# brianz98/A-Fortran-Electronic-Structure-Program

Measured on AMD Instinct MI355X. Metric: CCSD iter wall-time (s) + (T) wall-time (s); fp64 TFLOP/s vs MFMA peak, higher is better.
Workload: dtype f64; 1 GPU; cfg5: nocc=20 nvirt=200, synthetic hashed ERIs scale 0.005; step = 1 CCSD iteration (replicated) + full (T) over i<=j<=k sharded across ranks; nocc=20, nvirt=200, triples=1540, parallelism=(T) ijk-shard x1, CCSD replicas

## Files before the change

a-fortran-electronic-structure-program_amd/csrc/triples.hip:

```cpp
#include <algorithm>
#include <cmath>
#include <cstdio>
#include <cstdlib>
#include <cstring>
#include <unordered_map>

#include "ccsd.h"
#include "ccsd_so.h"
#include "tgemm.h"
#include "triples_orbit.h"

namespace afesp {

int64_t triples_count(int o) { return (int64_t)o * (o + 1) * (o + 2) / 6; }

__global__ __launch_bounds__(256) void triples_sum_kernel(double* out, const double* partial, int nblk)
{
    __shared__ double sm[4];
    const int q = blockIdx.x;
    const int per = (nblk + (int)gridDim.y - 1) / (int)gridDim.y;
    const int lo = (int)blockIdx.y * per, hi = min(nblk, lo + per);
    double s = 0.0;
    for (int b = lo + threadIdx.x; b < hi; b += blockDim.x) s += partial[(int64_t)q * nblk + b];
#pragma unroll
// ... 80 lines not shown
    for (int off = 32; off > 0; off >>= 1) s += __shfl_down(s, off, 64);
    if ((threadIdx.x & 63) == 0) sm[threadIdx.x >> 6] = s;
    __syncthreads();
    if (threadIdx.x == 0) {
        for (int q = 0; q < 4; ++q) partial[(int64_t)q * nblk_total + blockIdx.x] = 0.0;
        partial[(int64_t)2 * nblk_total + blockIdx.x] = sm[0] + sm[1] + sm[2] + sm[3] + (blockIdx.x == 0 ? 1.0 : 0.0);
    }
}

__global__ __launch_bounds__(256) void triples_build_vt_kernel(double* vt, double* vtT, const double* X, int64_t sb, int64_t sc, int64_t sk,
                                                             int64_t sd, const double* t2, int o, int v, int Kc)
{
    const int64_t n = (int64_t)Kc * v * v * o;
    for (int64_t x = (int64_t)blockIdx.x * blockDim.x + threadIdx.x; x < n; x += (int64_t)gridDim.x * blockDim.x) {
        const int kap = (int)(x % Kc);
        int64_t r = x / Kc;
        const int b = (int)(r % v);
        r /= v;
        const int c = (int)(r % v), k = (int)(r / v);
        double val = 0.0;
        if (kap < v) val = X[sb * b + sc * c + sk * k + sd * kap];
        else if (kap < v + o) val = t2[(kap - v) + (int64_t)o * (k + (int64_t)o * (b + (int64_t)v * c))];
        vt[x] = val;
        vtT[kap + (int64_t)Kc * (c + (int64_t)v * (b + (int64_t)v * k))] = val;
    }
}
__global__ __launch_bounds__(256) void triples_build_vt_tiled_kernel(double* vt, double* vtT, const double* X, int64_t sb, int64_t sk, int64_t sd,
                                                                   const double* t2, int o, int v, int Kc)
{
    __shared__ double tile[32][33];
    const int nkt = (Kc + 31) / 32, nct = (v + 31) / 32;
    int64_t blk = blockIdx.x;
    const int kap0 = (int)(blk % nkt) * 32;
    blk /= nkt;
    const int c0 = (int)(blk % nct) * 32;
    blk /= nct;
    const int b = (int)(blk % v), k = (int)(blk / v);
    const int tx = threadIdx.x & 31, ty = threadIdx.x >> 5;
#pragma unroll
    for (int r = 0; r < 4; ++r) {
        const int kap = kap0 + ty + 8 * r, c = c0 + tx;
        double val = 0.0;
        if (c < v) {
            if (kap < v) val = X[sb * b + c + sk * k + sd * kap];
            else if (kap < v + o) val = t2[(kap - v) + (int64_t)o * (k + (int64_t)o * (b + (int64_t)v * c))];
        }
        tile[ty + 8 * r][tx] = val;
    }
    __syncthreads();
#pragma unroll
    for (int r = 0; r < 4; ++r) {
        const int kap = kap0 + tx, c = c0 + ty + 8 * r;
        if (kap < Kc && c < v) {
            const double val = tile[tx][ty + 8 * r];
            vt[kap + (int64_t)Kc * (b + (int64_t)v * (c + (int64_t)v * k))] = val;
            vtT[kap + (int64_t)Kc * (c + (int64_t)v * (b + (int64_t)v * k))] = val;
        }
    }
}
__global__ __launch_bounds__(256) void triples_build_tt_kernel(double* tt, const double* t2, const double* Y, int64_t si, int64_t sj, int64_t sa,
                                                             int64_t sl, int o, int v, int Kc)
{
    const int64_t n = (int64_t)Kc * v * o * o;
    for (int64_t x = (int64_t)blockIdx.x * blockDim.x + threadIdx.x; x < n; x += (int64_t)gridDim.x * blockDim.x) {
        const int kap = (int)(x % Kc);
        int64_t r = x / Kc;
        const int a = (int)(r % v);
        r /= v;
        const int j = (int)(r % o), i = (int)(r / o);
        double val = 0.0;
        if (kap < v) val = t2[i + (int64_t)o * (j + (int64_t)o * (a + (int64_t)v * kap))];
        else if (kap < v + o) val = -Y[si * i + sj * j + sa * a + sl * (kap - v)];
        tt[x] = val;
    }
}

struct TriplesPlan {
    int o = 0, v = 0;
    int64_t t_begin = -1, t_end = -1, nb = 0;
    int norb = 0;
    bool cr = false;
    int mode = 0;
    int sblock = 0;
    int64_t epoch = -1;
    struct Group { int r; int64_t start, N; int q = 0; int64_t koffA = 0, koffB = 0; };
    struct Chunk { int nt; int64_t meta_off, tab_off, ntab; std::vector<Group> groups;
                   int64_t gdesc_off = 0; int total_tiles = 0, max_ntiles = 0;
                   int64_t gdesc_diag_off = 0; int ngroups_diag = 0, total_tiles_diag = 0, max_ntiles_diag = 0, ngroups_off = 0;
                   int64_t ncol_off = 0, ncol_diag = 0; bool split_diag = false;
                   int64_t tg_off = 0, tab32_off = 0; int tg_ngroups = 0, tg_tiles = 0, tg_max_ntiles = 0; };
    std::vector<Chunk> chunks;
    int64_t* tables = nullptr;
    int64_t off_k = 0, off_Am = 0, off_Cm = 0;
    TripleMeta* meta = nullptr;
    int* orbits = nullptr;
    GettGroup* gdesc = nullptr;
    bool use_tg = false;
    TgGroup* tgdesc = nullptr;
    uint32_t* tables32 = nullptr;
    bool c_pairs = false;
    int k_block = 0;
    int64_t k_pool_gib = -1, k_split_tiles = 0;
    bool k_one_pool = false;
    double* pool0 = nullptr;
};

static std::vector<int64_t> assemble_pool(Context& cx, int64_t nblocks, int64_t vp3, double** pool0)
{
    const size_t bb = (size_t)vp3 * sizeof(double);
    struct Piece { char* base; int64_t n; };
    std::vector<Piece> have;
    int64_t cap = 0;
    for (int i = 0;; ++i) {
        auto it = cx.cache.find("t_xpool" + std::to_string(i));
        if (it == cx.cache.end()) break;
        have.push_back({(char*)it->second.first, (int64_t)(it->second.second / bb)});
        cap += have.back().n;
    }
    if (cap < nblocks) {
        if (!have.empty()) cx.drop_scratch("t_xpool");
        have.clear();
        int64_t need = nblocks;
        for (int i = 0; need > 0; ++i) {
            const std::string name = "t_xpool" + std::to_string(i);
            size_t got = 0;
            void* q = cx.arena.take_largest((size_t)need * bb, (size_t)need * bb + (size_t)need * bb / 4, &got);
            if (!q) q = cx.arena.take_largest((size_t)std::min<int64_t>(need, 8) * bb, (size_t)need * bb, &got);
            int64_t k;
            if (q) {
                k = std::min<int64_t>(need, (int64_t)(got / bb));
                cx.cache[name] = {q, got};
            } else {
                k = need;
                q = cx.scratch(name, k * vp3);
            }
            have.push_back({(char*)q, k});
            need -= k;
        }
    }
    *pool0 = (double*)have[0].base;
    std::vector<int64_t> off;
    off.reserve((size_t)nblocks);
    for (const Piece& pc : have)
        for (int64_t b = 0; b < pc.n && (int64_t)off.size() < nblocks; ++b)
            off.push_back((int64_t)((pc.base - have[0].base) / (ptrdiff_t)sizeof(double)) + b * vp3);
    return off;
}

static bool fused_use_tg(int o, int v);

static TriplesPlan* plan_for(Context& cx, void*& slot, int o, int v, int64_t t_begin, int64_t t_end)
{
    TriplesPlan* p = (TriplesPlan*)slot;
    if (p && p->o == o && p->v == v && p->t_begin == t_begin && p->t_end == t_end && p->mode == 1 && p->epoch == cx.scratch_epoch &&
        p->use_tg == (fused_use_tg(o, v) && (((int64_t)v + o + 15) / 16 * 16) >= 2 * TG_BK))
        return p;
    delete p;
    p = new TriplesPlan();
    slot = p;
    const int64_t O = o, V = v, Kc = (V + O + 15) / 16 * 16;
    p->o = o; p->v = v; p->t_begin = t_begin; p->t_end = t_end; p->cr = false; p->mode = 1;
    p->use_tg = fused_use_tg(o, v) && Kc >= 2 * TG_BK;
    p->c_pairs = (v % 2) == 0;
    std::vector<uint32_t> tab32;
    if (p->use_tg)
        for (int64_t m = 0; m < V * V; ++m) tab32.push_back((uint32_t)(8 * Kc * m));
    const int64_t nt8 = (V + TT - 1) / TT, vp3 = nt8 * nt8 * nt8 * CUBE;
    const int64_t per = 3 * vp3 * (int64_t)sizeof(double);
    size_t mem_free = 0, mem_total = 0;
// ... 122 lines not shown
    cx.sync();
    p->epoch = cx.scratch_epoch;
    return p;
}

static int fused_block_size(int o, int v, bool cr, int64_t budget_bytes)
{
    (void)cr;
    const int64_t nt8 = (v + TT - 1) / TT, vp3 = nt8 * nt8 * nt8 * CUBE;
    const int64_t per_block = vp3 * (int64_t)sizeof(double);
    int smax = 1;
    while (smax < o && (int64_t)3 * (smax + 1) * (smax + 1) * (smax + 1) * per_block <= budget_bytes) ++smax;
    if (knobs().t_block > 0) return std::max(1, std::min(smax, knobs().t_block));
    const int smin = std::min(smax, std::max(1, (900 + v - 1) / v));
    auto fill = [&](int sz) { return (double)((int64_t)v * sz) / (double)((((int64_t)v * sz + 127) / 128) * 128); };
    int best = smin;
    for (int sz = smin + 1; sz <= std::min(smax, smin + 2); ++sz)
        if (fill(sz) > fill(best) + 0.02) best = sz;
    return best;
}

static int64_t device_pool_budget()
{
    size_t mem_free = 0, mem_total = 0;
    AFESP_HIP(hipMemGetInfo(&mem_free, &mem_total));
    if (knobs().t_pool_gib >= 0) return knobs().t_pool_gib << 30;
    return std::min<int64_t>((int64_t)64 << 30, (int64_t)(mem_total / 4));
}

static bool fused_use_tg(int o, int v)
{
    if (knobs().t_gemm_gett) return false;
    const int64_t O = o, V = v, Kc = (V + O + 15) / 16 * 16;
    return 8 * Kc * V * V < ((int64_t)1 << 32) && 8 * Kc * V * O * O < ((int64_t)1 << 32);
}

static TriplesPlan* plan_fused(Context& cx, void*& slot, int o, int v, int64_t t_begin, int64_t t_end, bool cr)
{
    TriplesPlan* p = (TriplesPlan*)slot;
    const bool use_tg = fused_use_tg(o, v);
    if (p && p->o == o && p->v == v && p->t_begin == t_begin && p->t_end == t_end && p->cr == cr && p->mode == 0 &&
        p->epoch == cx.scratch_epoch && p->use_tg == use_tg && p->k_block == knobs().t_block && p->k_pool_gib == knobs().t_pool_gib &&
        p->k_split_tiles == knobs().t_split_tiles && p->k_one_pool == knobs().t_one_pool)
        return p;
    delete p;
    p = new TriplesPlan();
    slot = p;
    const int64_t O = o, V = v, v2 = V * V, Kc = (V + O + 15) / 16 * 16;
    const int64_t nt8 = (V + TT - 1) / TT, vp3 = nt8 * nt8 * nt8 * CUBE;
    p->o = o; p->v = v; p->t_begin = t_begin; p->t_end = t_end; p->cr = cr; p->mode = 0; p->use_tg = use_tg;
    p->k_block = knobs().t_block; p->k_pool_gib = knobs().t_pool_gib; p->k_split_tiles = knobs().t_split_tiles; p->k_one_pool = knobs().t_one_pool;
    p->c_pairs = (v % 2) == 0;
    const int nk1 = (int)(Kc / TG_BK);
    std::vector<uint32_t> tab32;
    if (use_tg)
        for (int64_t m = 0; m < v2; ++m) tab32.push_back((uint32_t)(8 * Kc * m));
    const int sb = fused_block_size(o, v, cr, device_pool_budget());
    p->sblock = sb;
    const int nbk = (o + sb - 1) / sb;
    std::vector<int64_t> tab;
    p->off_k = 0;
    p->off_Am = (int64_t)tab.size();
    for (int64_t c = 0; c < V; ++c)
        for (int64_t b = 0; b < V; ++b) tab.push_back(Kc * (b + V * c));
    p->off_Cm = (int64_t)tab.size();
    for (int64_t c = 0; c < V; ++c)
        for (int64_t b = 0; b < V; ++b)
            tab.push_back(CUBE * nt8 * (b / TT) + TT * (b % TT) + CUBE * nt8 * nt8 * (c / TT) + TT * TT * (c % TT));
    std::vector<TripleMeta> metas;
    int64_t flat = 0, max_blocks = 1;
    int tm, tn, BM, BN;
    gett_grouped_tile((int)v2, true, &tm, &tn, &BM, &BN);
    const int mtiles = (int)((v2 + BM - 1) / BM);
    const int64_t split_min_tiles = knobs().t_split_tiles;
    {
        int64_t fl = 0;
        for (int I = 0; I < nbk; ++I)
            for (int J = I; J < nbk; ++J)
                for (int K = J; K < nbk; ++K) {
                    std::unordered_map<int64_t, int> seen;
                    for (int i = I * sb; i < std::min(o, (I + 1) * sb); ++i)
                        for (int j = std::max(i, J * sb); j < std::min(o, (J + 1) * sb); ++j)
                            for (int k = std::max(j, K * sb); k < std::min(o, (K + 1) * sb); ++k, ++fl) {
                                if (fl < t_begin || fl >= t_end) continue;
                                const int pq[3][3] = {{i, j, k}, {j, i, k}, {k, i, j}};
                                for (auto& b : pq) seen.emplace(((int64_t)b[0] * o + std::min(b[1], b[2])) * o + std::max(b[1], b[2]), 0);
                            }
                    max_blocks = std::max<int64_t>(max_blocks, (int64_t)seen.size());
                }
    }
    if (cr) {
        if (cx.cache.count("t_xpool0")) cx.drop_scratch("t_xpool");
    } else {
        cx.drop_scratch("t_mpool");
        if (cx.cache.count("t_xpool")) {
            cx.quiesce();
            cx.arena.put(cx.cache["t_xpool"].first);
            cx.cache.erase("t_xpool");
            ++cx.scratch_epoch;
        }
    }
    std::vector<int64_t> blk_off;
    if (cr || knobs().t_one_pool) {
        for (int64_t b = 0; b < max_blocks; ++b) blk_off.push_back(b * vp3);
        p->pool0 = nullptr;
    } else {
        blk_off = assemble_pool(cx, max_blocks, vp3, &p->pool0);
    }
    for (int I = 0; I < nbk; ++I)
        for (int J = I; J < nbk; ++J)
            for (int K = J; K < nbk; ++K) {
                std::vector<TripleMeta> cur;
                struct Blk { int p, q, r; int64_t buf; };
                std::vector<Blk> blks;
                std::unordered_map<int64_t, int64_t> seen;
                auto block_of = [&](int pp, int qq, int rr) {
                    if (qq > rr) std::swap(qq, rr);
                    const int64_t key = ((int64_t)pp * o + qq) * o + rr;
                    auto it = seen.find(key);
                    if (it != seen.end()) return it->second;
                    blks.push_back({pp, qq, rr, (int64_t)blks.size()});
                    seen.emplace(key, blks.back().buf);
                    return blks.back().buf;
                };
                for (int i = I * sb; i < std::min(o, (I + 1) * sb); ++i)
                    for (int j = std::max(i, J * sb); j < std::min(o, (J + 1) * sb); ++j)
                        for (int k = std::max(j, K * sb); k < std::min(o, (K + 1) * sb); ++k, ++flat) {
                            if (flat < t_begin || flat >= t_end) continue;
                            TripleMeta m;
                            m.i = i; m.j = j; m.k = k;
                            m.pad = (j == k ? 1 : 0) | (i == k ? 2 : 0) | (i == j ? 4 : 0);
                            m.mult = (i == j && j == k) ? 1.0 : (i == j || j == k) ? 3.0 : 6.0;
                            m.woff = 0;
                            for (int q = 0; q < 6; ++q) m.xoff[q] = 0;
                            m.xoff[0] = blk_off[(size_t)block_of(i, j, k)];
                            m.xoff[1] = blk_off[(size_t)block_of(j, i, k)];
                            m.xoff[5] = blk_off[(size_t)block_of(k, i, j)];
                            cur.push_back(m);
                        }
                if (cur.empty()) continue;
                TriplesPlan::Chunk ch;
                ch.nt = (int)cur.size();
                ch.meta_off = (int64_t)metas.size();
                metas.insert(metas.end(), cur.begin(), cur.end());
                if ((int64_t)blks.size() > max_blocks) throw Error(2, "triples plan: block count of a chunk exceeds the pool");
                std::vector<int64_t> hBn, hCn, hK;
                std::stable_sort(blks.begin(), blks.end(), [](const Blk& x, const Blk& y) { return x.q != y.q ? x.q < y.q : x.r < y.r; });
                for (size_t b0 = 0; b0 < blks.size();) {
                    const int q = blks[b0].q, r = blks[b0].r;
                    size_t b1 = b0;
                    while (b1 < blks.size() && blks[b1].q == q && blks[b1].r == r) ++b1;
                    const int64_t start = (int64_t)hBn.size();
                    for (size_t bi = b0; bi < b1; ++bi)
                        for (int64_t x = 0; x < V; ++x) {
                            hBn.push_back(Kc * (x + V * (q + O * blks[bi].p)));
                            hCn.push_back(CUBE * (x / TT) + x % TT + blk_off[(size_t)blks[bi].buf]);
                        }
                    b0 = b1;
                    TriplesPlan::Group g;
                    g.r = r; g.q = q; g.start = start; g.N = (int64_t)hBn.size() - start;
                    g.koffA = (int64_t)hK.size();
                    for (int64_t x = 0; x < Kc; ++x) hK.push_back(x);
                    for (int64_t x = 0; x < Kc; ++x) hK.push_back(Kc * v2 * O + Kc * v2 * ((int64_t)q - r) + x);
                    g.koffB = (int64_t)hK.size();
                    for (int64_t x = 0; x < Kc; ++x) hK.push_back(x);
                    for (int64_t x = 0; x < Kc; ++x) hK.push_back(Kc * V * ((int64_t)r - q) + x);
                    ch.groups.push_back(g);
                }
                int64_t diag_tiles = 0;
                for (const TriplesPlan::Group& g : ch.groups)
                    if (g.q == g.r) diag_tiles += mtiles * ((g.N + BN - 1) / BN);
                ch.split_diag = diag_tiles >= split_min_tiles;
                if (use_tg) ch.split_diag = nk1 >= 2;
                if (!ch.split_diag)
                    for (int t = 0; t < ch.nt; ++t) metas[ch.meta_off + t].pad = 0;
                ch.ntab = (int64_t)hBn.size();
                if (use_tg) {
                    ch.tab32_off = (int64_t)tab32.size();
                    for (int64_t x : hBn) tab32.push_back((uint32_t)(8 * x));
                }
                ch.tab_off = (int64_t)tab.size();
                tab.insert(tab.end(), hBn.begin(), hBn.end());
                tab.insert(tab.end(), hCn.begin(), hCn.end());
                const int64_t kbase = (int64_t)tab.size() - ch.tab_off;
                tab.insert(tab.end(), hK.begin(), hK.end());
                for (TriplesPlan::Group& g : ch.groups) { g.koffA += kbase; g.koffB += kbase; }
                p->chunks.push_back(std::move(ch));
            }
    p->nb = max_blocks;
    std::vector<int> orb;
    for (int A = 0; A < nt8; ++A)
        for (int B = A; B < nt8; ++B)
            for (int C = B; C < nt8; ++C) orb.push_back(A | (B << 10) | (C << 20));
    p->norb = (int)orb.size();
    if (metas.empty()) metas.push_back(TripleMeta());
    tab.resize(tab.size() + 128, 0);
    p->tables = (int64_t*)cx.scratch("t_tables", (int64_t)tab.size());
    p->meta = (TripleMeta*)cx.scratch("t_meta", (int64_t)(metas.size() * sizeof(TripleMeta) / sizeof(double) + 1));
    p->orbits = (int*)cx.scratch("t_orbits", (int64_t)orb.size() / 2 + 1);
    AFESP_HIP(hipMemcpyAsync(p->tables, tab.data(), tab.size() * sizeof(int64_t), hipMemcpyHostToDevice, cx.stream));
    AFESP_HIP(hipMemcpyAsync(p->meta, metas.data(), metas.size() * sizeof(TripleMeta), hipMemcpyHostToDevice, cx.stream));
    AFESP_HIP(hipMemcpyAsync(p->orbits, orb.data(), orb.size() * sizeof(int), hipMemcpyHostToDevice, cx.stream));
    std::vector<GettGroup> gd;
    for (TriplesPlan::Chunk& ch : p->chunks) {
        const int64_t* tabs = p->tables + ch.tab_off;
      for (int diag = 0; diag < 2; ++diag) {
        (diag ? ch.gdesc_diag_off : ch.gdesc_off) = (int64_t)gd.size();
        int tile = 0, ng = 0, mx = 0;
        int64_t ncol = 0;
        for (const TriplesPlan::Group& g : ch.groups) {
            if ((ch.split_diag && g.q == g.r) != (diag == 1)) continue;
            GettGroup d;
            d.a_off = Kc * v2 * g.r;
            d.offAk = tabs + g.koffA;
            d.offBk = tabs + g.koffB;
            d.offBn = tabs + g.start;
            d.offCn = tabs + ch.ntab + g.start;
            d.N = (int)g.N;
            d.ntiles = (int)((g.N + BN - 1) / BN);
            d.tile_start = tile;
            d.pad = 0;
            tile += mtiles * d.ntiles;
            mx = std::max(mx, d.ntiles);
            ncol += g.N;
            ++ng;
            gd.push_back(d);
        }
        GettGroup end{};
        end.tile_start = tile;
        gd.push_back(end);
        if (diag) { ch.total_tiles_diag = tile; ch.ngroups_diag = ng; ch.max_ntiles_diag = mx; ch.ncol_diag = ncol; }
        else { ch.total_tiles = tile; ch.ngroups_off = ng; ch.max_ntiles = mx; ch.ncol_off = ncol; }
      }
    }
    p->gdesc = (GettGroup*)cx.scratch("t_gdesc", (int64_t)(gd.size() * sizeof(GettGroup) / sizeof(double) + 1));
    AFESP_HIP(hipMemcpyAsync(p->gdesc, gd.data(), gd.size() * sizeof(GettGroup), hipMemcpyHostToDevice, cx.stream));
    std::vector<TgGroup> tg;
    if (use_tg) {
        tab32.resize(tab32.size() + 256, 0u);
        p->tables32 = (uint32_t*)cx.scratch("t_tables32", (int64_t)(tab32.size() / 2 + 1));
        AFESP_HIP(hipMemcpyAsync(p->tables32, tab32.data(), tab32.size() * sizeof(uint32_t), hipMemcpyHostToDevice, cx.stream));
        const int mt = (int)((v2 + TG_BM - 1) / TG_BM);
        for (TriplesPlan::Chunk& ch : p->chunks) {
            const int64_t* tabs = p->tables + ch.tab_off;
            ch.tg_off = (int64_t)tg.size();
            int mx = 0;
            for (const TriplesPlan::Group& g : ch.groups) mx = std::max(mx, (int)((g.N + TG_BN - 1) / TG_BN));
            const int gm = tgemm_group_m((int)v2, mx);
            int tile = 0;
            for (int pass = 0; pass < 2; ++pass)
            for (const TriplesPlan::Group& g : ch.groups) {
                const bool half = ch.split_diag && g.q == g.r;
                if (half != (pass == 1)) continue;
                TgGroup d;
                d.a1 = Kc * v2 * g.r;
                d.a2 = Kc * v2 * O + Kc * v2 * g.q;
                d.b1 = 0;
                d.b2 = Kc * V * ((int64_t)g.r - g.q);
                d.c0 = 0;
                d.colB = p->tables32 + ch.tab32_off + g.start;
                d.offCn = tabs + ch.ntab + g.start;
                d.N = (int)g.N;
                d.ntiles = (int)((g.N + TG_BN - 1) / TG_BN);
                d.tile_start = tile;
                d.nk1 = nk1;
                d.nk = half ? nk1 : 2 * nk1;
                d.inv_width = tgemm_inverse(gm * d.ntiles);
                if ((int64_t)mt * d.ntiles * gm * d.ntiles >= ((int64_t)1 << 32)) throw Error(2, "triples plan: tile walk out of range");
                tile += mt * d.ntiles;
                tg.push_back(d);
            }
            TgGroup end{};
            end.tile_start = tile;
            tg.push_back(end);
            ch.tg_ngroups = (int)ch.groups.size();
            ch.tg_tiles = tile;
            ch.tg_max_ntiles = mx;
        }
        p->tgdesc = (TgGroup*)cx.scratch("t_tgdesc", (int64_t)(tg.size() * sizeof(TgGroup) / sizeof(double) + 1));
        AFESP_HIP(hipMemcpyAsync(p->tgdesc, tg.data(), tg.size() * sizeof(TgGroup), hipMemcpyHostToDevice, cx.stream));
    }
    cx.sync();
    p->epoch = cx.scratch_epoch;
    return p;
}

static double fused_range_cost(int o, int v, int sb, int64_t b, int64_t e, int BM, int BN, int64_t split_min_tiles)
{
    const int64_t V = v, O = o, v2 = V * V, Kc = (V + O + 15) / 16 * 16;
    const int64_t nt8 = (V + TT - 1) / TT, vp3 = nt8 * nt8 * nt8 * CUBE;
    const int64_t mtiles = (v2 + BM - 1) / BM;
    const int nbk = (o + sb - 1) / sb;
    const double half_tile_s = 2.0 * BM * BN * (double)Kc / 58e12;
    const double triple_s = 3.0 * (double)vp3 * 8.0 / 3.9e12;
    double cost = 0.0;
    int64_t flat = 0;
    std::unordered_map<int64_t, int> npair;
    std::unordered_map<int64_t, char> seen;
    for (int I = 0; I < nbk && flat < e; ++I)
        for (int J = I; J < nbk && flat < e; ++J)
            for (int K = J; K < nbk && flat < e; ++K) {
                npair.clear();
                seen.clear();
                int64_t nt = 0;
                auto need = [&](int pp, int qq, int rr) {
                    if (qq > rr) std::swap(qq, rr);
                    if (seen.emplace(((int64_t)pp * o + qq) * o + rr, 1).second) ++npair[(int64_t)qq * o + rr];
                };
                for (int i = I * sb; i < std::min(o, (I + 1) * sb); ++i)
                    for (int j = std::max(i, J * sb); j < std::min(o, (J + 1) * sb); ++j)
                        for (int k = std::max(j, K * sb); k < std::min(o, (K + 1) * sb); ++k, ++flat) {
                            if (flat < b || flat >= e) continue;
                            ++nt;
                            need(i, j, k);
                            need(j, i, k);
                            need(k, i, j);
                        }
                if (nt == 0) continue;
                int64_t off = 0, diag = 0;
                for (const auto& g : npair) {
                    const int64_t tiles = mtiles * ((V * g.second + BN - 1) / BN);
                    (g.first / o == g.first % o ? diag : off) += tiles;
                }
                const double halves = 2.0 * (double)off + (diag >= split_min_tiles ? 1.0 : 2.0) * (double)diag;
                cost += std::max(halves, 512.0) * half_tile_s + (double)nt * triple_s + 40e-6;
            }
    return cost;
}

void triples_shard_bounds(int o, int v, bool cr, int world, int64_t* bounds)
{
    const int64_t V = v, nt = triples_count(o);
    int tm, tn, BM, BN;
    gett_grouped_tile((int)(V * V), true, &tm, &tn, &BM, &BN);
    const int sb = fused_block_size(o, v, cr, device_pool_budget());
    const int64_t split_min_tiles = knobs().t_split_tiles;
    auto cost = [&](int64_t b, int64_t e) { return fused_range_cost(o, v, sb, b, e, BM, BN, split_min_tiles); };
    bounds[0] = 0;
    if (cost(0, nt) < (double)world * cost(0, 1)) {
        for (int r = 1; r <= world; ++r) bounds[r] = nt * r / world;
        return;
    }
    for (int r = 0; r < world; ++r) {
        const int64_t b = bounds[r];
        if (r == world - 1 || b >= nt) { bounds[r + 1] = nt; continue; }
        const double target = cost(b, nt) / (double)(world - r);
        int64_t lo = b, hi = nt;
        while (lo < hi) {
            const int64_t mid = (lo + hi) / 2;
            if (cost(b, mid) >= target) hi = mid; else lo = mid + 1;
        }
        if (lo > b + 1 && target - cost(b, lo - 1) < cost(b, lo) - target) --lo;
        bounds[r + 1] = lo;
    }
}

int triples_block_size(int o, int v, bool cr) { return fused_block_size(o, v, cr, device_pool_budget()); }

void triples_plan_free(CCState& s)
{
    delete (TriplesPlan*)s.tplan;
    s.tplan = nullptr;
}

void ccsd_triples(Context& cx, CCState& s, int64_t t_begin, int64_t t_end, double* out_host, bool cr, bool want_d)
{
    if (cr) want_d = true;
    if (cr && !s.have_cr) throw Error(1, "ccsd_triples: completely renormalised mode needs ccsd_cr_intermediates first");
    if (!s.ready) throw Error(1, "ccsd_triples: no converged CCSD state in this context");
    const int o = s.o, v = s.v;
    const int64_t O = o, V = v, v2 = V * V, v3 = V * V * V;
    const int64_t nt8 = (V + TT - 1) / TT, vp3 = nt8 * nt8 * nt8 * CUBE;
    const int64_t Kc = (V + O + 15) / 16 * 16;
    t_begin = std::max<int64_t>(0, t_begin);
    t_end = std::min<int64_t>(triples_count(o), t_end);
    TriplesPlan* p = plan_fused(cx, s.tplan, s.o, s.v, t_begin, t_end, cr);
    if (knobs().t_debug)
        fprintf(stderr, "afesp (T): o %d v %d block %d chunks %zu kernel %s\n", o, v, p->sblock, p->chunks.size(), p->use_tg ? "tgemm" : "gett");
    Tensor vt = view(cx.scratch("t_vt", 2 * Kc * v2 * O), {Kc, V, V, O}), tt = view(cx.scratch("t_tt", Kc * V * O * O), {Kc, V, O, O});
    Tensor vtT = vt;
    vtT.d = vt.d + Kc * v2 * O;
    auto blocks = [](int64_t n) { return dim3((unsigned)std::min<int64_t>((n + 255) / 256, 65536)); };
    const bool ops_valid = cx.t_ops_owner == (const void*)&s && cx.t_ops_amp == s.amp_epoch && cx.t_ops_scratch == cx.scratch_epoch;
    if (!ops_valid) { cx.t_ops_ts = false; cx.t_ops_cr = -1; }
    if (!ops_valid) {
        const int64_t nblk = ((Kc + 31) / 32) * ((V + 31) / 32) * V * O;
        if (nblk < ((int64_t)1 << 31))
            AFESP_KLAUNCH(triples_build_vt_tiled_kernel, dim3((unsigned)nblk), dim3(256), 0, cx.stream, vt.d, vtT.d, s.v_vvov.d, V, v2,
                               v2 * O, s.t2.d, o, v, (int)Kc);
        else
            AFESP_KLAUNCH(triples_build_vt_kernel, blocks(Kc * v2 * O), dim3(256), 0, cx.stream, vt.d, vtT.d, s.v_vvov.d, V,
                               (int64_t)1, v2, v2 * O, s.t2.d, o, v, (int)Kc);
        AFESP_HIP(hipGetLastError());
        AFESP_KLAUNCH(triples_build_tt_kernel, blocks(Kc * V * O * O), dim3(256), 0, cx.stream, tt.d, s.t2.d, s.v_oovo.d, (int64_t)1, O,
                           O * O, O * O * V, o, v, (int)Kc);
        AFESP_HIP(hipGetLastError());
    }
    Tensor vs = view(cx.scratch("t_vs", v2 * O * O), {V, V, O, O});
    Tensor ts = view(cx.scratch("t_ts", v2 * O * O), {V, V, O, O});
    if (!ops_valid) permute_add(cx, 1.0, s.v_oovv, "pqxy", 0.0, vs, "xypq");
    if (want_d && !cx.t_ops_ts) {
        permute_add(cx, 1.0, s.t2, "pqxy", 0.0, ts, "xypq");
        cx.t_ops_ts = true;
    }
    Tensor vt2, tt2;
    double* Mpool = nullptr;
    if (cr) {
        vt2 = view(cx.scratch("t_vt2", 2 * Kc * v2 * O), {Kc, V, V, O});
        tt2 = view(cx.scratch("t_tt2", Kc * V * O * O), {Kc, V, O, O});
        Tensor vt2T = vt2;
        vt2T.d = vt2.d + Kc * v2 * O;
        if (cx.t_ops_cr != s.cr_epoch) {
            AFESP_KLAUNCH(triples_build_vt_kernel, blocks(Kc * v2 * O), dim3(256), 0, cx.stream, vt2.d, vt2T.d, s.I_vovv_pp.d, V * O,
                               v2 * O, V, (int64_t)1, s.t2.d, o, v, (int)Kc);
            AFESP_HIP(hipGetLastError());
            AFESP_KLAUNCH(triples_build_tt_kernel, blocks(Kc * V * O * O), dim3(256), 0, cx.stream, tt2.d, s.t2.d, s.I_ooov_pp.d, O,
                               (int64_t)1, O * O * O, O * O, o, v, (int)Kc);
            AFESP_HIP(hipGetLastError());
            cx.t_ops_cr = s.cr_epoch;
        }
        Mpool = cx.scratch("t_mpool", p->nb * vp3);
    }
    cx.t_ops_owner = (const void*)&s;
    cx.t_ops_amp = s.amp_epoch;
    cx.t_ops_scratch = cx.scratch_epoch;
    const int nq = cr ? 6 : want_d ? 4 : 2;
    const bool dbase = t_begin == 0 && want_d;
    double pub_seq = 0.0;
    double* pub = (p->chunks.size() == 1 && !dbase && (int64_t)p->norb * p->chunks[0].nt <= 8192) ? host_scalars_slot(cx, &pub_seq) : nullptr;
    if (!pub) k_fill(cx, cx.scal, 6, 0.0);
    TriplesIn in{s.e, s.t1.d, vs.d, ts.d, s.t2.d, o, v};
    double* Xpool = p->pool0 ? p->pool0 : cx.scratch("t_xpool", p->nb * vp3);
    int64_t max_nt = 1;
    for (const TriplesPlan::Chunk& ch : p->chunks) max_nt = std::max<int64_t>(max_nt, ch.nt);
    double* partial = cx.scratch("t_partial", 6 * std::max<int64_t>((int64_t)p->norb * max_nt, 512));
    double* sum_tmp = cx.scratch("t_sum_tmp", 6 * 128);
    std::vector<hipEvent_t> evs;
    auto stamp = [&]() {
        if (!cx.prof) return;
        hipEvent_t e;
        AFESP_HIP(hipEventCreate(&e));
        AFESP_HIP(hipEventRecord(e, cx.stream));
        evs.push_back(e);
    };
    for (const TriplesPlan::Chunk& ch : p->chunks) {
        stamp();
        {
            GettProblem gp;
            gp.A = vt.d;
            gp.B = tt.d;
            gp.C = Xpool;
            gp.offAm = p->tables + p->off_Am;
            gp.offAk = gp.offBk = gp.offBn = gp.offCn = nullptr;
            gp.offCm = p->tables + p->off_Cm;
            gp.M = (int)v2; gp.N = 0; gp.K = (int)(2 * Kc);
            gp.alpha = 1.0; gp.beta = 0.0;
            gp.nbatch = 1; gp.batchA = gp.batchB = gp.batchC = nullptr;
            gp.a_kcontig = gp.b_kcontig = true;
            gp.wide = true;
            GettProblem gm = gp;
            gm.A = vt2.d;
            gm.B = tt2.d;
            gm.C = Mpool;
            if (p->use_tg) {
                TgProblem tp{vt.d, tt.d, Xpool, p->tables32, p->tables + p->off_Cm, (int)v2, p->c_pairs, (int)((V + O - (Kc - TG_BK) + 3) / 4)};
                AFESP_HIP(tgemm_launch(tp, p->tgdesc + ch.tg_off, ch.tg_ngroups, ch.tg_tiles, ch.tg_max_ntiles, cx.stream, cx.tg));
                if (cr) {
                    TgProblem tm{vt2.d, tt2.d, Mpool, p->tables32, p->tables + p->off_Cm, (int)v2, p->c_pairs, (int)((V + O - (Kc - TG_BK) + 3) / 4)};
                    AFESP_HIP(tgemm_launch(tm, p->tgdesc + ch.tg_off, ch.tg_ngroups, ch.tg_tiles, ch.tg_max_ntiles, cx.stream, cx.tg));
                }
            } else {
            if (ch.ngroups_off > 0) {
                const GettGroup* gd = p->gdesc + ch.gdesc_off;
                AFESP_HIP(gett_launch_grouped(gp, gd, ch.ngroups_off, ch.total_tiles, ch.max_ntiles, cx.stream));
                if (cr) AFESP_HIP(gett_launch_grouped(gm, gd, ch.ngroups_off, ch.total_tiles, ch.max_ntiles, cx.stream));
            }
            if (ch.ngroups_diag > 0) {
                const GettGroup* gd = p->gdesc + ch.gdesc_diag_off;
                gp.K = gm.K = (int)Kc;
                AFESP_HIP(gett_launch_grouped(gp, gd, ch.ngroups_diag, ch.total_tiles_diag, ch.max_ntiles_diag, cx.stream));
                if (cr) AFESP_HIP(gett_launch_grouped(gm, gd, ch.ngroups_diag, ch.total_tiles_diag, ch.max_ntiles_diag, cx.stream));
            }
            }
            if (cx.prof) {
                cx.prof_gemm_kind = p->use_tg ? 1 : 0;
                for (const TriplesPlan::Group& g : ch.groups) {
                    const bool half = ch.split_diag && g.q == g.r;
                    if (p->use_tg) {
                        const double kexec = (double)(Kc - TG_BK) + ((V + O - (Kc - TG_BK) + 3) / 4 < 4 ? 12.0 : 16.0);
                        cx.prof_gemm_flop_padded += 2.0 * (double)((v2 + TG_BM - 1) / TG_BM * TG_BM) * (double)((g.N + TG_BN - 1) / TG_BN * TG_BN) *
                                                    kexec * (half ? 1.0 : 2.0);
                    } else {
                        int tm_, tn_, BM_, BN_;
                        gett_grouped_tile((int)v2, true, &tm_, &tn_, &BM_, &BN_);
                        cx.prof_gemm_flop_padded += 2.0 * (double)((v2 + BM_ - 1) / BM_ * BM_) * (double)((g.N + BN_ - 1) / BN_ * BN_) *
                                                    (double)Kc * (half ? 1.0 : 2.0);
                    }
                }
                cx.prof_gemm_launches += p->use_tg ? 1 : (ch.ngroups_off > 0) + (ch.ngroups_diag > 0);
                cx.prof_gemm_flop += 2.0 * (double)gp.M * (double)(2 * ch.ncol_off + ch.ncol_diag) * (double)(V + O);
            }
        }
        stamp();
        if (cr)
            AFESP_KLAUNCH((triples_orbit_kernel<true, true>), dim3(p->norb, ch.nt), dim3(256), 0, cx.stream, partial, Xpool, Mpool,
                               p->meta + ch.meta_off, p->orbits, in, p->norb * ch.nt);
        else if (!want_d)
            AFESP_KLAUNCH((triples_orbit_kernel<false, true, false>), dim3(p->norb, ch.nt), dim3(256), 0, cx.stream, partial, Xpool,
                               Mpool, p->meta + ch.meta_off, p->orbits, in, p->norb * ch.nt);
        else
            AFESP_KLAUNCH((triples_orbit_kernel<false, true>), dim3(p->norb, ch.nt), dim3(256), 0, cx.stream, partial, Xpool, Mpool,
                               p->meta + ch.meta_off, p->orbits, in, p->norb * ch.nt);
        AFESP_HIP(hipGetLastError());
        stamp();
        if (cx.prof) {
            cx.prof_orbit_launches += 1;
            cx.prof_orbit_bytes += 8.0 * 3.0 * (double)v3 * ch.nt;
        }
        if (pub) {
            AFESP_KLAUNCH(triples_sum_publish_kernel, dim3(1), dim3(256), 0, cx.stream, cx.scal, pub, pub_seq, partial, nq, p->norb * ch.nt);
            AFESP_HIP(hipGetLastError());
        } else {
            sum_partials(cx, cx.scal, partial, nq, p->norb * ch.nt, sum_tmp);
        }
    }
    if (dbase) {
        AFESP_KLAUNCH(triples_dbase_kernel, dim3(256), dim3(256), 0, cx.stream, partial, in, 256);
        AFESP_HIP(hipGetLastError());
        AFESP_KLAUNCH(triples_sum_kernel, dim3(4), dim3(256), 0, cx.stream, cx.scal, partial, 256);
        AFESP_HIP(hipGetLastError());
    }
    double* h = pub ? host_scalars_wait(cx, 6, pub_seq) : host_scalars(cx, 6);
    if (!evs.empty()) AFESP_HIP(hipEventSynchronize(evs.back()));
    for (size_t q = 0; q + 2 < evs.size(); q += 3) {
        float a = 0.f, b = 0.f;
        AFESP_HIP(hipEventElapsedTime(&a, evs[q], evs[q + 1]));
        AFESP_HIP(hipEventElapsedTime(&b, evs[q + 1], evs[q + 2]));
        cx.prof_gemm_ms += a;
        cx.prof_orbit_ms += b;
    }
    for (hipEvent_t e : evs) (void)hipEventDestroy(e);
    out_host[0] = h[0];
    out_host[1] = h[0] + h[1];
    if (!want_d) return;
    out_host[2] = h[2];
    out_host[3] = h[2] + h[3];
    if (cr) {
        out_host[4] = h[4];
        out_host[5] = h[4] + h[5];
    }
}

int64_t so_triples_count(int o) { return (int64_t)o * (o - 1) * (o - 2) / 6; }

void so_triples_plan_free(SOState& s)
{
    delete (TriplesPlan*)s.tplan;
    s.tplan = nullptr;
}

__global__ void so_levels_kernel(double* e_so, const double* e, int n2)
{
    const int x = blockIdx.x * blockDim.x + threadIdx.x;
    if (x < n2) e_so[x] = e[x / 2];
}

double so_triples(Context& cx, SOState& s, int64_t t_begin, int64_t t_end)
{
    if (!s.ready) throw Error(1, "ccsd_so_triples: no converged spin-orbital CCSD state in this context");
    if (s.fock && s.f_offdiag > 1e-8)
        throw Error(1, "ccsd_so_triples: the occupied-occupied / virtual-virtual Fock blocks of this state are not diagonal (largest off-diagonal "
                       "element " + std::to_string(s.f_offdiag) + "): (T) needs semicanonical orbitals");
    const int o = s.o, v = s.v;
    const int64_t O = o, V = v, v2 = V * V;
    const int64_t nt8 = (V + TT - 1) / TT, vp3 = nt8 * nt8 * nt8 * CUBE;
    const int64_t Kc = (V + O + 15) / 16 * 16;
    t_begin = std::max<int64_t>(0, t_begin);
    t_end = std::min<int64_t>(so_triples_count(o), t_end);
    k_fill(cx, cx.scal, 1, 0.0);
    if (t_end <= t_begin) return 0.0;
    TriplesPlan* p = plan_for(cx, s.tplan, o, v, t_begin, t_end);
    Tensor vt = view(cx.scratch("t_vt", Kc * v2 * O), {Kc, V, V, O}), tt = view(cx.scratch("t_tt", Kc * V * O * O), {Kc, V, O, O});
    Tensor vs = view(cx.scratch("t_vs", v2 * O * O), {V, V, O, O});
    double* e_so = cx.scratch("t_eso", O + V);
    const bool ops_valid = cx.t_ops_owner == (const void*)&s && cx.t_ops_amp == s.amp_epoch && cx.t_ops_scratch == cx.scratch_epoch;
    if (!ops_valid) {
    auto sub = [&](const Tensor& full, int64_t row0, int64_t nrows) {
        Tensor t = full;
        t.d = full.d + row0;
        t.dim[0] = nrows;
        return t;
    };
    if (Kc != V + O) {
        AFESP_HIP(hipMemsetAsync(vt.d, 0, sizeof(double) * Kc * v2 * O, cx.stream));
        AFESP_HIP(hipMemsetAsync(tt.d, 0, sizeof(double) * Kc * V * O * O, cx.stream));
    }
    permute_add(cx, 1.0, s.vovv, "fpbc", 0.0, sub(vt, 0, V), "fbcp");
    permute_add(cx, 1.0, s.t2, "mpcb", 0.0, sub(vt, V, O), "mbcp");
    permute_add(cx, 1.0, s.t2, "qraf", 0.0, sub(tt, 0, V), "farq");
    permute_add(cx, -1.0, s.ovoo, "maqr", 0.0, sub(tt, V, O), "marq");
// ... 65 lines not shown
```

a-fortran-electronic-structure-program_amd/csrc/triples_orbit.h:

```cpp
#pragma once
#include <hip/hip_runtime.h>
#include <stdint.h>

namespace afesp {

struct TripleMeta {
    int i, j, k, pad;
    double mult;
    int64_t xoff[6];
    int64_t woff;
};

struct TriplesIn {
    const double* e;
    const double* t1;
    const double* voovv_s;
    const double* t2_s;
    const double* t2;
    int o, v;
};

#ifdef AFESP_ORBIT_STAMPS
constexpr int ORB_SLOTS = 4096;
__device__ unsigned long long g_orbit_stamp[ORB_SLOTS * 16];
#define ORB_STAMP(k)                                                                                                          \
    {                                                                                                                         \
        const unsigned long long now_ = __builtin_amdgcn_s_memtime();                                                         \
        if (threadIdx.x == 0) g_orbit_stamp[((blockIdx.y * gridDim.x + blockIdx.x) % ORB_SLOTS) * 16 + (k)] = now_ - orb_last_; \
        orb_last_ = now_;                                                                                                     \
    }
#else
#define ORB_STAMP(k) {}
#endif

#ifndef AFESP_ORBIT_DEPTH
#define AFESP_ORBIT_DEPTH 0
#endif
constexpr int TT = 8;
constexpr int CUBE = TT * TT * TT;
constexpr int PATCH = TT * TT;

__host__ __device__ constexpr int sig(int s, int d)
{
    return s == 0 ? d : s == 1 ? (d == 0 ? 1 : d == 1 ? 0 : 2) : s == 2 ? 2 - d : s == 3 ? (d == 0 ? 0 : d == 1 ? 2 : 1)
                      : s == 4 ? (d + 1) % 3 : (d + 2) % 3;
}
__device__ __forceinline__ double rcp_nr(double x)
{
    double r = __builtin_amdgcn_rcp(x);
    r = __builtin_fma(__builtin_fma(-x, r, 1.0), r, r);
    r = __builtin_fma(__builtin_fma(-x, r, 1.0), r, r);
    return r;
}
__device__ __forceinline__ int cidx(int p0, int p1, int p2) { return ((p0 ^ p1 ^ p2) & 7) | (p1 << 3) | (p2 << 6); }

__host__ __device__ constexpr int orbit_term(bool fused, int idx) { return fused ? (idx == 0 ? 0 : idx == 1 ? 1 : 5) : idx; }

__host__ __device__ constexpr int compose(int q, int s)
{
    for (int r = 0; r < 6; ++r)
        if (sig(r, 0) == sig(q, sig(s, 0)) && sig(r, 1) == sig(q, sig(s, 1)) && sig(r, 2) == sig(q, sig(s, 2))) return r;
    return 0;
}

template <bool CR, bool FUSED, bool WANT_D = true>
__global__ __launch_bounds__(256, CR ? 2 : WANT_D ? 3 : 4) void triples_orbit_kernel(double* __restrict__ partial, const double* __restrict__ Xpool,
                                                            const double* __restrict__ Mpool,
                                                            const TripleMeta* __restrict__ meta,
                                                            const int* __restrict__ orbits, TriplesIn in, int nblk_total)
{
    __shared__ __attribute__((aligned(16))) double stage[6 * CUBE];
    __shared__ double vp[27 * PATCH];
    __shared__ double tp[WANT_D ? 27 * PATCH : 1];
    __shared__ double t1r[96];
    __shared__ int srcq[6][6];
    __shared__ double red[24];
#ifdef AFESP_ORBIT_STAMPS
    unsigned long long orb_last_ = __builtin_amdgcn_s_memtime();
#endif
    const TripleMeta m = meta[blockIdx.y];
    const int o = in.o, v = in.v, t = threadIdx.x;
    const int packed = orbits[blockIdx.x];
    const int tile[3] = {packed & 1023, (packed >> 10) & 1023, (packed >> 20) & 1023};
    if (t < 36) {
        const int s = t / 6, q = t % 6;
        int want[3];
        for (int d = 0; d < 3; ++d) want[d] = tile[sig(q, sig(s, d))];
        int found = 0;
        for (int r = 5; r >= 0; --r)
            if (tile[sig(r, 0)] == want[0] && tile[sig(r, 1)] == want[1] && tile[sig(r, 2)] == want[2]) found = r;
        srcq[s][q] = found;
    }
    const int64_t vv = (int64_t)v * v;
    const int l0 = t & 7, l1 = (t >> 3) & 7, l2h[2] = {t >> 6, (t >> 6) + 4};
    const int nt8 = (v + TT - 1) / TT;
    const int p0 = (2 * t) & 7, p1 = (t >> 2) & 7, p2 = t >> 5;
    const int sbase = (((p0 ^ p1 ^ p2) & 7) & ~1) | (p1 << 3) | (p2 << 6);
    const bool flip = ((p1 ^ p2) & 1) != 0;
    typedef double v2d_t __attribute__((ext_vector_type(2)));
    auto load_term = [&](const double* X, v2d_t (&xin)[6]) {
#pragma unroll
        for (int q = 0; q < 6; ++q) {
            const int T0 = tile[sig(q, 0)], T1 = tile[sig(q, 1)], T2 = tile[sig(q, 2)];
            const v2d_t x = *reinterpret_cast<const v2d_t*>(X + (int64_t)CUBE * (T0 + (int64_t)nt8 * (T1 + (int64_t)nt8 * T2)) + 2 * t);
            const int g0 = T0 * TT + p0;
            const bool rows = (T1 * TT + p1 < v) && (T2 * TT + p2 < v);
            xin[q][0] = (rows && g0 < v) ? x[0] : 0.0;
            xin[q][1] = (rows && g0 + 1 < v) ? x[1] : 0.0;
        }
    };
    auto park_term = [&](const v2d_t (&xin)[6]) {
#pragma unroll
        for (int q = 0; q < 6; ++q)
            *reinterpret_cast<v2d_t*>(&stage[q * CUBE + sbase]) = flip ? (v2d_t){xin[q][1], xin[q][0]} : xin[q];
    };
    constexpr int NT1 = FUSED ? 3 : 6;
    constexpr int NTERM = CR ? 2 * NT1 : NT1;
    constexpr int DEPTH = AFESP_ORBIT_DEPTH > 0 ? (AFESP_ORBIT_DEPTH < NT1 ? AFESP_ORBIT_DEPTH : NT1) : CR ? 3 : 2;
    v2d_t xin[DEPTH][6];
#pragma unroll
    for (int s2 = 0; s2 < DEPTH; ++s2) load_term(Xpool + m.xoff[orbit_term(FUSED, s2)], xin[s2]);
    const int occ[3] = {m.i, m.j, m.k};
    const int pairp[3] = {m.j, m.i, m.i}, pairq[3] = {m.k, m.k, m.j};
    {
        const int g = __builtin_amdgcn_readfirstlane(t >> 6), loc = t & 63;
#pragma unroll
        for (int i = 0; i < 5; ++i) {
            const int P = g + 4 * i;
            if (P < 18) {
                const int pr = P / 6, pi = P % 6;
                const int sx = pi < 2 ? 0 : pi < 4 ? 1 : 2, sy = pi == 0 ? 1 : pi == 1 ? 2 : pi == 2 ? 0 : pi == 3 ? 2 : pi == 4 ? 0 : 1;
                const int gx = tile[sx] * TT + (loc & 7), gy = tile[sy] * TT + (loc >> 3);
                const bool ok = gx < v && gy < v;
                const int64_t off = (ok ? gx + (int64_t)v * gy : 0) + vv * (pairp[pr] + (int64_t)o * pairq[pr]);
                const int dst = (pr * 9 + sx * 3 + sy) * PATCH + loc;
                const double a = in.voovv_s[off];
                vp[dst] = ok ? a : 0.0;
                if (WANT_D) {
                    const double b = in.t2_s[off];
                    tp[dst] = ok ? b : 0.0;
                }
            }
        }
    }
    if (t < 72) {
        const int oc = t / 24, sl = (t / 8) % 3, l = t & 7, g = tile[sl] * TT + l;
        t1r[t] = g < v ? in.t1[occ[oc] + o * g] : 0.0;
    } else if (t < 96) {
        const int sl = (t - 72) / 8, l = t & 7, g = tile[sl] * TT + l;
        t1r[t] = in.e[(g < v ? g : 0) + o];
    }
    const double* evl = t1r + 72;
    double wreg[12];
    double mreg[CR ? 12 : 1];
#pragma unroll
    for (int r = 0; r < 12; ++r) wreg[r] = 0.0;
#pragma unroll
    for (int r = 0; r < (CR ? 12 : 1); ++r) mreg[r] = 0.0;
#pragma unroll
    for (int s2 = 0; s2 < NTERM; ++s2) {
        const int s = orbit_term(FUSED, s2 % NT1);
        const int sT = s == 0 ? 3 : s == 1 ? 4 : 2;
        const bool sym = FUSED && ((m.pad >> (s2 % NT1)) & 1);
        if (s2 == 0) ORB_STAMP(0)
        __syncthreads();
        park_term(xin[s2 % DEPTH]);
        if (s2 + DEPTH < NTERM)
            load_term((s2 + DEPTH < NT1 ? Xpool : Mpool) + m.xoff[orbit_term(FUSED, (s2 + DEPTH) % NT1)], xin[s2 % DEPTH]);
        __syncthreads();
        if (s2 < 3) ORB_STAMP(1 + 2 * s2)
#define ORB_READ(sg) stage[srcq[sg][q] * CUBE + cidx(l[sig(q, sig(sg, 0))], l[sig(q, sig(sg, 1))], l[sig(q, sig(sg, 2))])]
        double xr[12];
        if (FUSED && sym) {
#pragma unroll
            for (int r = 0; r < 12; ++r) {
                const int q = r >> 1;
                const int l[3] = {l0, l1, l2h[r & 1]};
                xr[r] = ORB_READ(s) + ORB_READ(sT);
            }
        } else {
#pragma unroll
            for (int r = 0; r < 12; ++r) {
                const int q = r >> 1;
                const int l[3] = {l0, l1, l2h[r & 1]};
                xr[r] = ORB_READ(s);
            }
        }
#undef ORB_READ
#pragma unroll
        for (int r = 0; r < 12; ++r) {
            if (s2 < NT1) wreg[r] += xr[r];
            else mreg[CR ? r : 0] += xr[r];
        }
        if (s2 < 3) ORB_STAMP(2 + 2 * s2)
    }
    const double eo = in.e[m.i] + in.e[m.j] + in.e[m.k];
    constexpr int NQ = CR ? 6 : WANT_D ? 4 : 2;
    double acc[NQ];
#pragma unroll
    for (int q = 0; q < NQ; ++q) acc[q] = 0.0;
#pragma unroll
    for (int h = 0; h < 2; ++h) {
        int l2v = l2h[h];
        if (h == 1) asm volatile("" : "+v"(l2v) : "v"(acc[0]), "v"(acc[NQ - 1]));
        const int l[3] = {l0, l1, l2v};
        const bool live = tile[0] * TT + l[0] < v && tile[1] * TT + l[1] < v && tile[2] * TT + l[2] < v;
        const double D = eo - evl[l[0]] - evl[TT + l[1]] - evl[2 * TT + l[2]];
        const double rD = rcp_nr(3.0 * D);
        const double r3D = live ? rD : 0.0;
        double t1v[3][3], Z[6], Y[WANT_D ? 6 : 1];
#pragma unroll
        for (int oc = 0; oc < 3; ++oc)
#pragma unroll
            for (int c = 0; c < 3; ++c) t1v[oc][c] = t1r[oc * 24 + c * TT + l[c]];
        {
            double V[3][3][3];
#pragma unroll
            for (int pr = 0; pr < 3; ++pr)
#pragma unroll
                for (int cx = 0; cx < 3; ++cx)
#pragma unroll
                    for (int cy = 0; cy < 3; ++cy)
                        if (cx != cy) V[pr][cx][cy] = vp[(pr * 9 + cx * 3 + cy) * PATCH + l[cx] + TT * l[cy]];
#pragma unroll
            for (int q = 0; q < 6; ++q) {
                const int s0 = sig(q, 0), s1 = sig(q, 1), s2 = sig(q, 2);
                Z[q] = t1v[0][s0] * V[0][s1][s2] + t1v[1][s1] * V[1][s0][s2] + t1v[2][s2] * V[2][s0][s1];
            }
        }
        if (WANT_D) {
            int lt[3] = {l[0], l[1], l[2]};
            asm volatile("" : "+v"(lt[0]), "+v"(lt[1]), "+v"(lt[2]) : "v"(Z[0]), "v"(Z[1]), "v"(Z[2]), "v"(Z[3]), "v"(Z[4]), "v"(Z[5]));
            double T2[3][3][3];
#pragma unroll
            for (int pr = 0; pr < 3; ++pr)
#pragma unroll
                for (int cx = 0; cx < 3; ++cx)
#pragma unroll
                    for (int cy = 0; cy < 3; ++cy)
                        if (cx != cy) T2[pr][cx][cy] = tp[(pr * 9 + cx * 3 + cy) * PATCH + lt[cx] + TT * lt[cy]];
#pragma unroll
            for (int q = 0; q < 6; ++q) {
                const int s0 = sig(q, 0), s1 = sig(q, 1), s2 = sig(q, 2);
                Y[q] = t1v[0][s0] * t1v[1][s1] * t1v[2][s2] + t1v[0][s0] * T2[0][s1][s2] + t1v[1][s1] * T2[1][s0][s2] +
                       t1v[2][s2] * T2[2][s0][s1];
            }
        }
#pragma unroll
        for (int q = 0; q < 6; ++q) {
            const double w = wreg[2 * q + h];
#define BAR3(A) (4.0 * A(q) + A(compose(q, 4)) + A(compose(q, 5)) - 2.0 * (A(compose(q, 3)) + A(compose(q, 1)) + A(compose(q, 2))))
#define W_AT(r) wreg[2 * (r) + h]
// ... 181 lines not shown
```

Measured before the change: 59.74 TFLOP/s.

## Skip i=j=k triples and reuse staged orbit terms for duplicate occupied indices

Drops fully diagonal (i=j=k) triples from the plan, partitioning and pool sizing, since their contribution is treated as zero. In the fused orbit kernel, triples with i==j or j==k now skip loading and staging the duplicate term: the already-parked shared-memory stage is reused and the register prefetch pipeline is shifted. This removes redundant global loads and barrier pairs for degenerate triples, at the cost of more complex per-block control flow and pointer selection. It also guards against empty host-to-device copies and adjusts partition cost and debug output.

```diff
diff --git a/a-fortran-electronic-structure-program_amd/csrc/triples.hip b/a-fortran-electronic-structure-program_amd/csrc/triples.hip
--- a/a-fortran-electronic-structure-program_amd/csrc/triples.hip
+++ b/a-fortran-electronic-structure-program_amd/csrc/triples.hip
@@ -186,9 +186,11 @@
     bool cr = false;
     int mode = 0;
     int sblock = 0;
+    int nblock_triples = 0;
     int64_t epoch = -1;
     struct Group { int r; int64_t start, N; int q = 0; int64_t koffA = 0, koffB = 0; };
-    struct Chunk { int nt; int64_t meta_off, tab_off, ntab; std::vector<Group> groups;
+    struct Chunk { int nt; int ndup = 0;
+                   int64_t meta_off, tab_off, ntab; std::vector<Group> groups;
                    int64_t gdesc_off = 0; int total_tiles = 0, max_ntiles = 0;
                    int64_t gdesc_diag_off = 0; int ngroups_diag = 0, total_tiles_diag = 0, max_ntiles_diag = 0, ngroups_off = 0;
                    int64_t ncol_off = 0, ncol_diag = 0; bool split_diag = false;
@@ -477,7 +479,7 @@
                     for (int i = I * sb; i < std::min(o, (I + 1) * sb); ++i)
                         for (int j = std::max(i, J * sb); j < std::min(o, (J + 1) * sb); ++j)
                             for (int k = std::max(j, K * sb); k < std::min(o, (K + 1) * sb); ++k, ++fl) {
-                                if (fl < t_begin || fl >= t_end) continue;
+                                if (fl < t_begin || fl >= t_end || (i == j && j == k)) continue;
                                 const int pq[3][3] = {{i, j, k}, {j, i, k}, {k, i, j}};
                                 for (auto& b : pq) seen.emplace(((int64_t)b[0] * o + std::min(b[1], b[2])) * o + std::max(b[1], b[2]), 0);
                             }
@@ -518,14 +520,18 @@
                     seen.emplace(key, blks.back().buf);
                     return blks.back().buf;
                 };
+                bool touched = false;
                 for (int i = I * sb; i < std::min(o, (I + 1) * sb); ++i)
                     for (int j = std::max(i, J * sb); j < std::min(o, (J + 1) * sb); ++j)
                         for (int k = std::max(j, K * sb); k < std::min(o, (K + 1) * sb); ++k, ++flat) {
                             if (flat < t_begin || flat >= t_end) continue;
+                            touched = true;
+                            if (i == j && j == k) continue;
                             TripleMeta m;
                             m.i = i; m.j = j; m.k = k;
                             m.pad = (j == k ? 1 : 0) | (i == k ? 2 : 0) | (i == j ? 4 : 0);
-                            m.mult = (i == j && j == k) ? 1.0 : (i == j || j == k) ? 3.0 : 6.0;
+                            m.pad |= (i == j ? ORB_DUP01 : 0) | (j == k ? ORB_DUP12 : 0);
+                            m.mult = (i == j || j == k) ? 3.0 : 6.0;
                             m.woff = 0;
                             for (int q = 0; q < 6; ++q) m.xoff[q] = 0;
                             m.xoff[0] = blk_off[(size_t)block_of(i, j, k)];
@@ -533,9 +539,11 @@
                             m.xoff[5] = blk_off[(size_t)block_of(k, i, j)];
                             cur.push_back(m);
                         }
+                p->nblock_triples += touched ? 1 : 0;
                 if (cur.empty()) continue;
                 TriplesPlan::Chunk ch;
                 ch.nt = (int)cur.size();
+                for (const TripleMeta& m : cur) ch.ndup += (m.pad & (ORB_DUP01 | ORB_DUP12)) ? 1 : 0;
                 ch.meta_off = (int64_t)metas.size();
                 metas.insert(metas.end(), cur.begin(), cur.end());
                 if ((int64_t)blks.size() > max_blocks) throw Error(2, "triples plan: block count of a chunk exceeds the pool");
@@ -568,7 +576,7 @@
                 ch.split_diag = diag_tiles >= split_min_tiles;
                 if (use_tg) ch.split_diag = nk1 >= 2;
                 if (!ch.split_diag)
-                    for (int t = 0; t < ch.nt; ++t) metas[ch.meta_off + t].pad = 0;
+                    for (int t = 0; t < ch.nt; ++t) metas[ch.meta_off + t].pad &= ~7;
                 ch.ntab = (int64_t)hBn.size();
                 if (use_tg) {
                     ch.tab32_off = (int64_t)tab32.size();
@@ -629,7 +637,8 @@
       }
     }
     p->gdesc = (GettGroup*)cx.scratch("t_gdesc", (int64_t)(gd.size() * sizeof(GettGroup) / sizeof(double) + 1));
-    AFESP_HIP(hipMemcpyAsync(p->gdesc, gd.data(), gd.size() * sizeof(GettGroup), hipMemcpyHostToDevice, cx.stream));
+    if (!gd.empty())
+        AFESP_HIP(hipMemcpyAsync(p->gdesc, gd.data(), gd.size() * sizeof(GettGroup), hipMemcpyHostToDevice, cx.stream));
     std::vector<TgGroup> tg;
     if (use_tg) {
         tab32.resize(tab32.size() + 256, 0u);
@@ -673,7 +682,8 @@
             ch.tg_max_ntiles = mx;
         }
         p->tgdesc = (TgGroup*)cx.scratch("t_tgdesc", (int64_t)(tg.size() * sizeof(TgGroup) / sizeof(double) + 1));
-        AFESP_HIP(hipMemcpyAsync(p->tgdesc, tg.data(), tg.size() * sizeof(TgGroup), hipMemcpyHostToDevice, cx.stream));
+        if (!tg.empty())
+            AFESP_HIP(hipMemcpyAsync(p->tgdesc, tg.data(), tg.size() * sizeof(TgGroup), hipMemcpyHostToDevice, cx.stream));
     }
     cx.sync();
     p->epoch = cx.scratch_epoch;
@@ -705,7 +715,7 @@
                 for (int i = I * sb; i < std::min(o, (I + 1) * sb); ++i)
                     for (int j = std::max(i, J * sb); j < std::min(o, (J + 1) * sb); ++j)
                         for (int k = std::max(j, K * sb); k < std::min(o, (K + 1) * sb); ++k, ++flat) {
-                            if (flat < b || flat >= e) continue;
+                            if (flat < b || flat >= e || (i == j && j == k)) continue;
                             ++nt;
                             need(i, j, k);
                             need(j, i, k);
@@ -732,7 +742,7 @@
     const int64_t split_min_tiles = knobs().t_split_tiles;
     auto cost = [&](int64_t b, int64_t e) { return fused_range_cost(o, v, sb, b, e, BM, BN, split_min_tiles); };
     bounds[0] = 0;
-    if (cost(0, nt) < (double)world * cost(0, 1)) {
+    if (nt < 2 || cost(0, nt) < (double)world * cost(1, 2)) {
         for (int r = 1; r <= world; ++r) bounds[r] = nt * r / world;
         return;
     }
@@ -771,7 +781,8 @@
     t_end = std::min<int64_t>(triples_count(o), t_end);
     TriplesPlan* p = plan_fused(cx, s.tplan, s.o, s.v, t_begin, t_end, cr);
     if (knobs().t_debug)
-        fprintf(stderr, "afesp (T): o %d v %d block %d chunks %zu kernel %s\n", o, v, p->sblock, p->chunks.size(), p->use_tg ? "tgemm" : "gett");
+        fprintf(stderr, "afesp (T): o %d v %d block %d chunks %d kernel %s launched %zu\n", o, v, p->sblock, p->nblock_triples,
+                p->use_tg ? "tgemm" : "gett", p->chunks.size());
     Tensor vt = view(cx.scratch("t_vt", 2 * Kc * v2 * O), {Kc, V, V, O}), tt = view(cx.scratch("t_tt", Kc * V * O * O), {Kc, V, O, O});
     Tensor vtT = vt;
     vtT.d = vt.d + Kc * v2 * O;
@@ -820,7 +831,7 @@
     cx.t_ops_amp = s.amp_epoch;
     cx.t_ops_scratch = cx.scratch_epoch;
     const int nq = cr ? 6 : want_d ? 4 : 2;
-    const bool dbase = t_begin == 0 && want_d;
+    const bool dbase = t_begin == 0 && t_end > 0 && want_d;
     double pub_seq = 0.0;
     double* pub = (p->chunks.size() == 1 && !dbase && (int64_t)p->norb * p->chunks[0].nt <= 8192) ? host_scalars_slot(cx, &pub_seq) : nullptr;
     if (!pub) k_fill(cx, cx.scal, 6, 0.0);
@@ -910,7 +921,7 @@
         stamp();
         if (cx.prof) {
             cx.prof_orbit_launches += 1;
-            cx.prof_orbit_bytes += 8.0 * 3.0 * (double)v3 * ch.nt;
+            cx.prof_orbit_bytes += 8.0 * (double)v3 * (3.0 * ch.nt - ch.ndup);
         }
         if (pub) {
             AFESP_KLAUNCH(triples_sum_publish_kernel, dim3(1), dim3(256), 0, cx.stream, cx.scal, pub, pub_seq, partial, nq, p->norb * ch.nt);
diff --git a/a-fortran-electronic-structure-program_amd/csrc/triples_orbit.h b/a-fortran-electronic-structure-program_amd/csrc/triples_orbit.h
--- a/a-fortran-electronic-structure-program_amd/csrc/triples_orbit.h
+++ b/a-fortran-electronic-structure-program_amd/csrc/triples_orbit.h
@@ -3,6 +3,9 @@
 #include <stdint.h>
 
 namespace afesp {
+
+constexpr int ORB_DUP01 = 8;
+constexpr int ORB_DUP12 = 16;
 
 struct TripleMeta {
     int i, j, k, pad;
@@ -61,6 +64,23 @@
     for (int r = 0; r < 6; ++r)
         if (sig(r, 0) == sig(q, sig(s, 0)) && sig(r, 1) == sig(q, sig(s, 1)) && sig(r, 2) == sig(q, sig(s, 2))) return r;
     return 0;
+}
+
+__host__ __device__ constexpr bool orbit_skip(int dup, int nt1, int s2) { return dup != 0 && s2 % nt1 == dup; }
+__host__ __device__ constexpr int orbit_pos(int dup, int nt1, int s2)
+{
+    int k = 0;
+    for (int x = 0; x < s2; ++x) k += orbit_skip(dup, nt1, x) ? 0 : 1;
+    return k;
+}
+__host__ __device__ constexpr int orbit_staged(int dup, int nt1, int k)
+{
+    int s2 = 0;
+    for (;; ++s2) {
+        if (orbit_skip(dup, nt1, s2)) continue;
+        if (k-- == 0) break;
+    }
+    return s2;
 }
 
 template <bool CR, bool FUSED, bool WANT_D = true>
@@ -117,9 +137,23 @@
     constexpr int NT1 = FUSED ? 3 : 6;
     constexpr int NTERM = CR ? 2 * NT1 : NT1;
     constexpr int DEPTH = AFESP_ORBIT_DEPTH > 0 ? (AFESP_ORBIT_DEPTH < NT1 ? AFESP_ORBIT_DEPTH : NT1) : CR ? 3 : 2;
+    constexpr int NSTAGE_DUP = NTERM - (CR ? 2 : 1);
+    const int dup = !FUSED ? 0 : (m.pad & ORB_DUP01) ? 1 : (m.pad & ORB_DUP12) ? 2 : 0;
+    const int64_t* __restrict__ xoff = meta[blockIdx.y].xoff;
+    auto term_ptr = [&](int s2) __attribute__((always_inline)) { return (s2 < NT1 ? Xpool : Mpool) + xoff[orbit_term(FUSED, s2 % NT1)]; };
+    auto staged_ptr = [&](int k) __attribute__((always_inline)) -> const double* {
+        const double* P0 = k < NTERM ? term_ptr(k) : nullptr;
+        if (!FUSED) return P0;
+        const double* P1 = k < NSTAGE_DUP ? term_ptr(orbit_staged(1, NT1, k)) : nullptr;
+        const double* P2 = k < NSTAGE_DUP ? term_ptr(orbit_staged(2, NT1, k)) : nullptr;
+        return dup == 1 ? P1 : dup == 2 ? P2 : P0;
+    };
     v2d_t xin[DEPTH][6];
 #pragma unroll
-    for (int s2 = 0; s2 < DEPTH; ++s2) load_term(Xpool + m.xoff[orbit_term(FUSED, s2)], xin[s2]);
+    for (int k = 0; k < DEPTH; ++k) {
+        const double* P = staged_ptr(k);
+        if (k < NSTAGE_DUP || P) load_term(P, xin[k]);
+    }
     const int occ[3] = {m.i, m.j, m.k};
     const int pairp[3] = {m.j, m.i, m.i}, pairq[3] = {m.k, m.k, m.j};
     {
@@ -163,11 +197,33 @@
         const int sT = s == 0 ? 3 : s == 1 ? 4 : 2;
         const bool sym = FUSED && ((m.pad >> (s2 % NT1)) & 1);
         if (s2 == 0) ORB_STAMP(0)
-        __syncthreads();
-        park_term(xin[s2 % DEPTH]);
-        if (s2 + DEPTH < NTERM)
-            load_term((s2 + DEPTH < NT1 ? Xpool : Mpool) + m.xoff[orbit_term(FUSED, (s2 + DEPTH) % NT1)], xin[s2 % DEPTH]);
-        __syncthreads();
+        if (FUSED && s2 % NT1 != 0 && dup == s2 % NT1) {
+            const int k = orbit_pos(s2 % NT1, NT1, s2);
+            v2d_t first[6];
+#pragma unroll
+            for (int q = 0; q < 6; ++q) first[q] = xin[s2 % DEPTH][q];
+#pragma unroll
+            for (int d = DEPTH - 1; d >= 1; --d)
+                if (k + d < NSTAGE_DUP)
+#pragma unroll
+                    for (int q = 0; q < 6; ++q) xin[(s2 + 1 + d) % DEPTH][q] = xin[(s2 + d) % DEPTH][q];
+            if (k < NSTAGE_DUP)
+#pragma unroll
+                for (int q = 0; q < 6; ++q) xin[(s2 + 1) % DEPTH][q] = first[q];
+        } else {
+            __syncthreads();
+            park_term(xin[s2 % DEPTH]);
+            const double* P0 = s2 + DEPTH < NTERM ? term_ptr(s2 + DEPTH) : nullptr;
+            const double* P = P0;
+            if (FUSED) {
+                const int k1 = orbit_pos(1, NT1, s2) + DEPTH, k2 = orbit_pos(2, NT1, s2) + DEPTH;
+                const double* P1 = k1 < NSTAGE_DUP ? term_ptr(orbit_staged(1, NT1, k1 < NSTAGE_DUP ? k1 : 0)) : nullptr;
+                const double* P2 = k2 < NSTAGE_DUP ? term_ptr(orbit_staged(2, NT1, k2 < NSTAGE_DUP ? k2 : 0)) : nullptr;
+                P = dup == 1 ? P1 : dup == 2 ? P2 : P0;
+            }
+            if (s2 + DEPTH < NTERM && P) load_term(P, xin[s2 % DEPTH]);
+            __syncthreads();
+        }
         if (s2 < 3) ORB_STAMP(1 + 2 * s2)
 #define ORB_READ(sg) stage[srcq[sg][q] * CUBE + cidx(l[sig(q, sig(sg, 0))], l[sig(q, sig(sg, 1))], l[sig(q, sig(sg, 2))])]
         double xr[12];
```

Measured after the change: 59.66 TFLOP/s. No clear change (-0.1%).
